# S-Taichiii/diffusion-model

Hardware: AMD Instinct MI355X
Metric: denoising steps/sec (CFG, T=1000, 32x32x4 latent, B=64) (higher is better)
Workload: dtype f32 (GEMMs: fp32 operands split fp16 hi+lo on the matrix cores, fp32 accumulate); 1 GPU; config 2: UnetCondWithGeomHead CFG=3.0 denoising step, B=64, 32x32x4, T=1000; global_batch=64, T=1000, parallelism=sample-sharded x1 (no per-step collective)

## Files before the change

diffusion-model_amd/dmx/csrc/igemm_wino.h:

```cpp
#pragma once
#include "common.h"
#include "igemm.h"
#include "igemm_x3.h"
#include "source.h"

namespace dmx {

#ifndef DMX_DIAG
#define DMX_DIAG 0
#endif
#if DMX_DIAG
constexpr int WSTAMP_SLOTS = 32, WSTAMP_BLOCKS = 2048;
__device__ unsigned long long g_wstamp[WSTAMP_SLOTS * WSTAMP_BLOCKS * 5];
DMX_DEV void wstamp(int slot, int k) {
  if (threadIdx.x == 0 && slot >= 0 && slot < WSTAMP_SLOTS) {
    const int b = (blockIdx.z * gridDim.y + blockIdx.y) * gridDim.x + blockIdx.x;
    if (b < WSTAMP_BLOCKS) {
      unsigned long long* q = g_wstamp + ((size_t)slot * WSTAMP_BLOCKS + b) * 5;
      q[k] = __builtin_amdgcn_s_memtime();
      if (k == 0) q[4] = ((unsigned long long)__builtin_amdgcn_s_getreg((20 << 0) | (0 << 6) | (3 << 11)) << 32) |
                         (unsigned)__builtin_amdgcn_s_getreg((4 << 0) | (0 << 6) | (31 << 11));
    }
  }
}
#define WSTAMP(k) wstamp(P.dslot, k)
#else
#define WSTAMP(k)
#endif

DMX_DEV double wino_u(const double (&g)[3][3], int i, int j) {
  double r[3];
#pragma unroll
  for (int b = 0; b < 3; ++b) {
    const double a0 = g[0][b], a1 = g[1][b], a2 = g[2][b];
    r[b] = i == 0 ? a0 : i == 1 ? 0.5 * (a0 + a1 + a2) : i == 2 ? 0.5 * (a0 - a1 + a2) : a2;
  }
  return j == 0 ? r[0] : j == 1 ? 0.5 * (r[0] + r[1] + r[2]) : j == 2 ? 0.5 * (r[0] - r[1] + r[2]) : r[2];
}

static __global__ void wino_pack_kernel(const float* B, int kpad, int cin, int cout, float scale, _Float16* uh,
                                        _Float16* ul) {
  const int NB = cout / 32, KK = cin / 16;
  const size_t total = (size_t)16 * NB * KK * 64;
  for (size_t q = (size_t)blockIdx.x * blockDim.x + threadIdx.x; q < total; q += (size_t)gridDim.x * blockDim.x) {
    const int lane = (int)(q & 63);
    const size_t f = q >> 6;
    const int kk = (int)(f % KK), nb = (int)((f / KK) % NB), xi = (int)(f / ((size_t)KK * NB));
    const int co = 32 * nb + (lane & 31), c0 = 16 * kk + 8 * (lane >> 5);
    half8 h, l;
#pragma unroll
    for (int e = 0; e < 8; ++e) {
      double g[3][3];
#pragma unroll
      for (int t = 0; t < 9; ++t) g[t / 3][t % 3] = (double)B[(size_t)co * kpad + (size_t)t * cin + c0 + e];
      const float u = (float)(wino_u(g, xi >> 2, xi & 3) * (double)scale);
      const _Float16 hh = (_Float16)u;
      h[e] = hh;
      l[e] = (_Float16)(u - (float)hh);
    }
    *reinterpret_cast<half8*>(uh + q * 8) = h;
    *reinterpret_cast<half8*>(ul + q * 8) = l;
  }
}

template <int W, int GNA, int EPI = EPI_STATS, int X1 = 0>
__global__ __launch_bounds__(512) void wino_kernel(const X3Params P) {
  static_assert(EPI == EPI_STATS || EPI == EPI_PARTIAL, "Winograd epilogues");
  static_assert(W == 32 || W == 16 || W == 8 || W == 4, "Winograd conv: image width 4, 8, 16 or 32");
  static_assert(W != 4 || GNA == 0, "W = 4: no GroupNorm-on-load instances");
  const IgemmParams& p = P.g;
  constexpr int TW = W / 2;
  constexpr int SPB = W == 8 ? 4 : W == 4 ? 16 : 1;
  constexpr int TPS = 64 / SPB;
  constexpr int HRS = (W == 32 ? 8 : W) + 2;
  constexpr int PS = W == 8 ? 11 : HRS;
  constexpr int HR = SPB * PS, HC = W + 2;
  constexpr int RP = W == 32 ? 88 : W == 16 ? 46 : W == 8 ? 26 : 18;
  constexpr int SQ = W == 4 ? 218 * 4 : PS * 8 * RP;
  constexpr int HBUF = SPB * SQ;
  constexpr bool RING0 = W == 4;
  constexpr int CK = 16;
  constexpr int NPC = RING0 ? SPB * W * W * (CK / 4) : HR * HC * (CK / 4);
  constexpr int NPI = (NPC + 511) / 512;
  static_assert(!RING0 || NPC % 512 == 0, "W = 4: interior pieces must fill whole thread rounds");
  constexpr int EPP = 34;
  constexpr int EPF = 16 * 32 * EPP;
  constexpr int LDSF = 2 * HBUF + 1024 > EPF ? 2 * HBUF + 1024 : EPF;
  __shared__ __attribute__((aligned(16))) float lds[LDSF];

  WSTAMP(0);
  const int tid = threadIdx.x, lane = tid & 63;
  const int wid = __builtin_amdgcn_readfirstlane(tid >> 6);
  const int wi = wid >> 1, jp = wid & 1;
  int mt, nt, bz;
  xcd_tile(mt, nt, bz);
  const int WA = p.W;
  const int BPS = W == 32 ? (p.H + 7) >> 3 : 1;
  const int HW = p.H * WA, C = p.src.C;
  const int nsmp = W == 32 ? mt / BPS : mt * SPB;
  const int band = W == 32 ? mt - nsmp * BPS : 0;
  const int y0 = 8 * band;
  const int nsamp = p.M / HW;
  const int nch_all = C / CK;
  const int cbeg = EPI == EPI_PARTIAL ? bz * p.ksplit : 0;
  const int nch = EPI == EPI_PARTIAL ? min(p.ksplit, nch_all - cbeg) : nch_all;

  int hoff[NPI], hls[NPI];
#pragma unroll
  for (int k = 0; k < NPI; ++k) {
    const int e = tid + 512 * k;
    const int h = e >> 2, q = e & 3;
    int hrow, hcol;
    if constexpr (RING0) {
      hrow = h / HC;
      hcol = h - hrow * HC;
    } else if constexpr (W == 32) {
      const int pr = (h >> 1) % 17, m = h & 1;
      hrow = (h >> 1) / 17;
      hcol = pr < 8 ? pr + 8 * m : pr < 16 ? 8 + pr + 8 * m : 32 + m;
    } else {
      const int t = (h >> 1) / HC;
      hcol = (h >> 1) - t * HC;
      hrow = 2 * t + (h & 1);
    }
    const int sh = RING0 ? h >> 4 : hrow / PS;
    const int ry = RING0 ? ((h >> 2) & 3) + 1 : hrow - sh * PS;
    const int hx = RING0 ? (h & 3) + 1 : hcol;
    const int y = y0 + ry - 1, x = hx - 1;
    const bool ok = e < NPC && ry < HRS && y >= 0 && y < p.H && x >= 0 && x < WA && nsmp + sh < nsamp;
    hoff[k] = ok ? ((((nsmp + sh) * p.H + y) * WA + x) * C + q * 4) : -1;
    hls[k] = e < NPC ? (sh * SQ + (ry * 2 + (hx & 1)) * RP * 4 + (hx >> 1) * 20 + q * 4) : 2 * HBUF + (tid & 255) * 4;
  }
  const __amdgpu_buffer_rsrc_t rA = rsrc_of(p.src.src0, P.a_bytes);
  const __amdgpu_buffer_rsrc_t rRes = rsrc_of(GNA == 2 ? (const void*)P.gn_res : (const void*)p.src.src0, P.a_bytes);

  __shared__ float2 gst_s[SPB];
  if constexpr (GNA) {
    __shared__ double gr1[4], gr2[4];
    for (int sp = 0; sp < SPB; ++sp) {
      if (tid < 256 && nsmp + sp < nsamp) {
        const float2* rp = P.gn_rowpart + (size_t)(nsmp + sp) * P.gn_cnt;
        double s1 = 0.0, s2 = 0.0;
        for (int i = tid; i < P.gn_cnt; i += 256) {
          const float2 q = rp[i];
          s1 += (double)q.x;
          s2 += (double)q.y;
        }
        s1 = wave_sum_dpp(s1);
        s2 = wave_sum_dpp(s2);
        if ((tid & 63) == 0) {
          gr1[tid >> 6] = s1;
          gr2[tid >> 6] = s2;
        }
      }
      __syncthreads();
      if (tid == 0) {
        const double cntd = (double)HW * (double)C;
        const double mean = ((gr1[0] + gr1[1]) + (gr1[2] + gr1[3])) / cntd;
        double var = ((gr2[0] + gr2[1]) + (gr2[2] + gr2[3])) / cntd - mean * mean;
        var = var < 0.0 ? 0.0 : var;
        gst_s[sp] = make_float2((float)mean, (float)(1.0 / sqrt(var + 1e-5)));
      }
      __syncthreads();
    }
  }

  floatx4 ha[NPI];
  floatx4 hr[GNA == 2 ? NPI : 1];
  auto load_halo = [&](int c) {
#pragma unroll
    for (int k = 0; k < NPI; ++k) {
      const int off = hoff[k] >= 0 ? (hoff[k] + (cbeg + c) * CK) * 4 : kOOB;
      ha[k] = bload_f4(rA, off, 0);
      if constexpr (GNA == 2) hr[k] = bload_f4(rRes, off, 0);
    }
  };
  auto store_halo = [&](int buf, int c) {
    float* hb = lds + buf * HBUF;
    floatx4 ggam = {0.f, 0.f, 0.f, 0.f}, gbet = {0.f, 0.f, 0.f, 0.f};
    if constexpr (GNA) {
      const int ch = (cbeg + c) * CK + (tid & 3) * 4;
      ggam = ld4(P.gn_gamma + ch);
      gbet = ld4(P.gn_beta + ch);
    }
#pragma unroll
    for (int k = 0; k < NPI; ++k) {
      floatx4 v = ha[k];
      if constexpr (GNA) {
        const float2 gst = gst_s[SPB == 1 ? 0 : min(hls[k] / SQ, SPB - 1)];
        v = gn_apply4v(v, gst, ggam, gbet, GNA == 1 ? 1 : 0);
        if constexpr (GNA == 2) {
#pragma unroll
          for (int j = 0; j < 4; ++j) v[j] = gelu(hr[k][j] + v[j]);
        }
        if (hoff[k] < 0) v = floatx4{0.f, 0.f, 0.f, 0.f};
      }
      *reinterpret_cast<floatx4*>(hb + hls[k]) = v;
    }
  };

  const int xi0 = 4 * wi + 2 * jp;
  const int NB = p.Cout / 32, KK = C / 16;
  const __amdgpu_buffer_rsrc_t rUh = rsrc_of(P.Uh, P.u_bytes), rUl = rsrc_of(P.Ul, P.u_bytes);
  int ub[2][2];
#pragma unroll
  for (int q = 0; q < 2; ++q)
#pragma unroll
    for (int n = 0; n < 2; ++n) ub[q][n] = (((xi0 + q) * NB + 2 * nt + n) * KK) * 1024;
  const int voff = lane * 16;
  half8 bh[2][2], bl[2][2];
  int cnext = 0;
  auto load_b = [&](int q, int n, int c) {
    const int cc = c < 0 ? cnext : c;
    bh[q][n] = bload_h8(rUh, voff, ub[q][n] + (cbeg + cc) * 1024);
    if constexpr (!X1) bl[q][n] = bload_h8(rUl, voff, ub[q][n] + (cbeg + cc) * 1024);
  };

  const int ra = wi == 0 ? 0 : wi == 2 ? 2 : 1;
  const int rb = wi == 0 ? 2 : wi == 2 ? 1 : wi == 1 ? 2 : 3;
  const float sr = wi == 1 ? 1.f : -1.f;
  const int cp = jp ? 2 : 0, cq = jp ? 1 : 2, cs = jp ? 3 : 1;
  const float sb = jp ? -1.f : 1.f;
  auto coff = [&](int col) { return (col & 1) * RP * 4 + (col >> 1) * 20; };
  const int oa = ra * 8 * RP, ob = rb * 8 * RP;
  const int op = coff(cp), oq = coff(cq), os = coff(cs);
  const int fr = lane & 31, fh = lane >> 5;
  int tb[2];
#pragma unroll
  for (int mb = 0; mb < 2; ++mb) {
    const int t = 32 * mb + fr, st = t / TPS, tt = t - st * TPS, ty = tt / TW, tx = tt - ty * TW;
    tb[mb] = st * SQ + 2 * ty * 8 * RP + tx * 20 + 8 * fh;
  }
  half8 ah[2][2], al[2][2];
  auto build = [&](int buf, int mb) {
    const float* hb = lds + buf * HBUF + tb[mb];
    unsigned vh[2][4], vl[2][4];
#pragma unroll
    for (int h = 0; h < 2; ++h) {
      floatx4 T[3];
      const int oc[3] = {op, oq, os};
#pragma unroll
      for (int k = 0; k < 3; ++k) {
        const floatx4 da = *reinterpret_cast<const floatx4*>(hb + oa + oc[k] + 4 * h);
        const floatx4 db = *reinterpret_cast<const floatx4*>(hb + ob + oc[k] + 4 * h);
#pragma unroll
        for (int e = 0; e < 4; ++e) T[k][e] = fmaf(db[e], sr, da[e]);
      }
#pragma unroll
      for (int e = 0; e < 4; e += 2) {
        const float a0 = T[0][e] - T[1][e], a1 = T[0][e + 1] - T[1][e + 1];
        const float b0 = fmaf(T[2][e], sb, T[1][e]), b1 = fmaf(T[2][e + 1], sb, T[1][e + 1]);
        if constexpr (X1) {
          vh[0][2 * h + e / 2] = __builtin_bit_cast(unsigned, __builtin_convertvector((f32x2){a0, a1}, half2v));
          vh[1][2 * h + e / 2] = __builtin_bit_cast(unsigned, __builtin_convertvector((f32x2){b0, b1}, half2v));
        } else {
          split2u(a0, a1, vh[0][2 * h + e / 2], vl[0][2 * h + e / 2]);
          split2u(b0, b1, vh[1][2 * h + e / 2], vl[1][2 * h + e / 2]);
        }
      }
    }
#pragma unroll
    for (int q = 0; q < 2; ++q) {
      ah[mb][q] = __builtin_bit_cast(half8, (u32x4){vh[q][0], vh[q][1], vh[q][2], vh[q][3]});
      if constexpr (!X1) al[mb][q] = __builtin_bit_cast(half8, (u32x4){vl[q][0], vl[q][1], vl[q][2], vl[q][3]});
    }
  };

  floatx16 acc[2][2][2];
#pragma unroll
  for (int q = 0; q < 2; ++q)
#pragma unroll
    for (int i = 0; i < 2; ++i)
#pragma unroll
      for (int j = 0; j < 2; ++j)
#pragma unroll
        for (int r = 0; r < 16; ++r) acc[q][i][j][r] = 0.f;

  if constexpr (RING0) {
    for (int i = tid; i < 2 * HBUF / 4; i += 512) *reinterpret_cast<floatx4*>(lds + 4 * i) = floatx4{0.f, 0.f, 0.f, 0.f};
  }
  load_halo(0);
  if constexpr (RING0) __syncthreads();
  store_halo(0, 0);
  load_halo(min(1, nch - 1));
  __builtin_amdgcn_sched_barrier(0);
#pragma unroll
  for (int q = 0; q < 2; ++q)
#pragma unroll
    for (int n = 0; n < 2; ++n) load_b(q, n, 0);
  __syncthreads();
  WSTAMP(1);

  auto mfmas = [&](int i, bool reload) {
#pragma unroll
    for (int q = 0; q < 2; ++q)
#pragma unroll
      for (int n = 0; n < 2; ++n) {
        if constexpr (!X1) {
          acc[q][i][n] = __builtin_amdgcn_mfma_f32_32x32x16_f16(al[i][q], bh[q][n], acc[q][i][n], 0, 0, 0);
          acc[q][i][n] = __builtin_amdgcn_mfma_f32_32x32x16_f16(ah[i][q], bl[q][n], acc[q][i][n], 0, 0, 0);
        }
        acc[q][i][n] = __builtin_amdgcn_mfma_f32_32x32x16_f16(ah[i][q], bh[q][n], acc[q][i][n], 0, 0, 0);
        if (reload) {
          load_b(q, n, -1);
          __builtin_amdgcn_sched_barrier(0x0086);
        }
      }
  };
  if constexpr (GNA == 0) {
  constexpr int NM = X1 ? 4 : 12;
  floatx4 pda[2][3], pdb[2][3], pT[3];
  u32x4 pah[2][2], pal[2][2];
  auto p_read = [&](int buf, int mb, int h) {
    const float* hb = lds + buf * HBUF + tb[mb];
    const int oc[3] = {op, oq, os};
#pragma unroll
    for (int k = 0; k < 3; ++k) {
      pda[h][k] = *reinterpret_cast<const floatx4*>(hb + oa + oc[k] + 4 * h);
      pdb[h][k] = *reinterpret_cast<const floatx4*>(hb + ob + oc[k] + 4 * h);
    }
  };
  auto p_T = [&](int h) {
#pragma unroll
    for (int k = 0; k < 3; ++k)
#pragma unroll
      for (int e = 0; e < 4; ++e) pT[k][e] = fmaf(pdb[h][k][e], sr, pda[h][k][e]);
  };
  auto p_V = [&](int mb, int h, int e) {
    const float a0 = pT[0][e] - pT[1][e], a1 = pT[0][e + 1] - pT[1][e + 1];
    const float b0 = fmaf(pT[2][e], sb, pT[1][e]), b1 = fmaf(pT[2][e + 1], sb, pT[1][e + 1]);
    const int j = 2 * h + e / 2;
    if constexpr (X1) {
      pah[mb][0][j] = __builtin_bit_cast(unsigned, __builtin_convertvector((f32x2){a0, a1}, half2v));
      pah[mb][1][j] = __builtin_bit_cast(unsigned, __builtin_convertvector((f32x2){b0, b1}, half2v));
    } else {
      unsigned h0, l0, h1, l1;
      split2u(a0, a1, h0, l0);
      split2u(b0, b1, h1, l1);
      pah[mb][0][j] = h0;
      pal[mb][0][j] = l0;
      pah[mb][1][j] = h1;
      pal[mb][1][j] = l1;
    }
  };
  auto p_piece = [&](int s, int buf, int mb) {
    if constexpr (X1) {
      if (s == 0) { p_read(buf, mb, 0); p_read(buf, mb, 1); }
      if (s == 1) { p_T(0); p_V(mb, 0, 0); p_V(mb, 0, 2); }
      if (s == 2) { p_T(1); p_V(mb, 1, 0); p_V(mb, 1, 2); }
    } else {
      if (s == 0) p_read(buf, mb, 0);
      if (s == 3) { p_T(0); p_read(buf, mb, 1); }
      if (s == 4) p_V(mb, 0, 0);
      if (s == 5) p_V(mb, 0, 2);
      if (s == 6) p_T(1);
      if (s == 7) p_V(mb, 1, 0);
      if (s == 8) p_V(mb, 1, 2);
    }
  };
  auto p_mfma = [&](int i, int s) {
    const int pr = X1 ? 2 : s % 3, qn = X1 ? s : s / 3, q = qn >> 1, n = qn & 1;
    const half8 A = __builtin_bit_cast(half8, pr == 0 ? pal[i][q] : pah[i][q]);
    const half8 Bf = pr == 1 ? bl[q][n] : bh[q][n];
    acc[q][i][n] = __builtin_amdgcn_mfma_f32_32x32x16_f16(A, Bf, acc[q][i][n], 0, 0, 0);
  };
  p_read(0, 0, 0);
  p_T(0);
  p_read(0, 0, 1);
  p_V(0, 0, 0);
  p_V(0, 0, 2);
  p_T(1);
  p_V(0, 1, 0);
  p_V(0, 1, 2);
  constexpr bool LATE = GNA == 2 || (W != 32 && GNA == 1);
  auto iter = [&](int c, auto last) {
    store_halo((c + 1) & 1, min(c + 1, nch - 1));
    if constexpr (!LATE) load_halo(min(c + 2, nch - 1));
    __builtin_amdgcn_sched_barrier(0);
#pragma unroll
    for (int sl = 0; sl < NM; ++sl) {
      p_mfma(0, sl);
      p_piece(sl, c & 1, 1);
      __builtin_amdgcn_sched_barrier(0);
    }
    __syncthreads();
    if constexpr (LATE) load_halo(min(c + 2, nch - 1));
    cnext = min(c + 1, nch - 1);
    __builtin_amdgcn_sched_barrier(0);
#pragma unroll
    for (int sl = 0; sl < NM; ++sl) {
      p_mfma(1, sl);
      if constexpr (!decltype(last)::value) p_piece(sl, (c + 1) & 1, 0);
      if (X1 || sl % 3 == 2) {
        const int qn = X1 ? sl : sl / 3;
        load_b(qn >> 1, qn & 1, -1);
      }
      __builtin_amdgcn_sched_barrier(0);
    }
  };
  for (int c = 0; c < nch - 1; ++c) iter(c, std::false_type{});
  iter(nch - 1, std::true_type{});
  } else {
  for (int c = 0; c < nch; ++c) {
    store_halo((c + 1) & 1, min(c + 1, nch - 1));
    constexpr bool LATE = GNA == 2 || (W != 32 && GNA == 1);
    if constexpr (!LATE) {
      load_halo(min(c + 2, nch - 1));
      __builtin_amdgcn_sched_barrier(0x0086);
    }
    build(c & 1, 0);
    mfmas(0, false);
    if constexpr (LATE) {
      load_halo(min(c + 2, nch - 1));
      __builtin_amdgcn_sched_barrier(0x0086);
    }
    build(c & 1, 1);
    cnext = min(c + 1, nch - 1);
    mfmas(1, true);
    __syncthreads();
  }
  }

  __syncthreads();
  WSTAMP(2);
  const int HW16 = BPS * 64 / SPB / 4, nseg = p.Cout / 32;
  const int tile0 = band * 64;
  const int cc = tid & 31, tp = tid >> 5;
#pragma unroll
  for (int mb = 0; mb < 2; ++mb)
#pragma unroll
    for (int n = 0; n < 2; ++n) {
#pragma unroll
      for (int q = 0; q < 2; ++q)
#pragma unroll
        for (int k = 0; k < 4; ++k) {
          floatx4 v;
#pragma unroll
          for (int e = 0; e < 4; ++e) v[e] = acc[q][mb][n][4 * k + e] * P.inv_scale;
          float* e = &lds[((xi0 + q) * 32 + fr) * EPP + 8 * k + 4 * fh];
          *reinterpret_cast<f32x2*>(e) = f32x2{v[0], v[1]};
          *reinterpret_cast<f32x2*>(e + 2) = f32x2{v[2], v[3]};
        }
      __syncthreads();
      float m[16][2];
#pragma unroll
      for (int xi = 0; xi < 16; ++xi) {
        const f32x2 v = *reinterpret_cast<const f32x2*>(&lds[(xi * 32 + cc) * EPP + 2 * tp]);
        m[xi][0] = v.x;
        m[xi][1] = v.y;
      }
      const int col = 64 * nt + 32 * n + cc;
      const float bias = (EPI == EPI_STATS && p.bias != nullptr) ? p.bias[col] : 0.f;
      float* dst = EPI == EPI_PARTIAL ? p.partial + (size_t)bz * p.M * p.Cout : p.out;
      float s1 = 0.f, s2 = 0.f;
#pragma unroll
      for (int e = 0; e < 2; ++e) {
        float z[4][2];
#pragma unroll
        for (int i = 0; i < 4; ++i) {
          z[i][0] = (m[4 * i][e] + m[4 * i + 1][e]) + m[4 * i + 2][e];
          z[i][1] = (m[4 * i + 1][e] - m[4 * i + 2][e]) - m[4 * i + 3][e];
        }
        const int t = 32 * mb + 2 * tp + e, st = t / TPS, tt = t - st * TPS, ty = tt / TW, tx = tt - ty * TW;
#pragma unroll
        for (int r = 0; r < 2; ++r)
#pragma unroll
          for (int s = 0; s < 2; ++s) {
            const float y = (r == 0 ? (z[0][s] + z[1][s]) + z[2][s] : (z[1][s] - z[2][s]) - z[3][s]) + bias;
            const int oy = y0 + 2 * ty + r, ox = 2 * tx + s;
            const bool in = oy < p.H && ox < WA;
            if (nsmp + st < nsamp && in)
              __builtin_nontemporal_store(y, &dst[(((size_t)(nsmp + st) * p.H + oy) * WA + ox) * p.Cout + col]);
            const float yv = in ? y : 0.f;
            s1 += yv;
            s2 += yv * yv;
          }
      }
      if constexpr (EPI == EPI_STATS) {
        s1 = wave_sum_dpp(s1);
        s2 = wave_sum_dpp(s2);
      }
      if (EPI == EPI_STATS && lane == 0) {
        const int t = 32 * mb + 4 * wid, st = t / TPS, g = (tile0 + t - st * TPS) / 4;
        if (nsmp + st < nsamp) p.rowpart[((size_t)(nsmp + st) * HW16 + g) * nseg + 2 * nt + n] = make_float2(s1, s2);
      }
      __syncthreads();
    }
  WSTAMP(3);
}

}
```

Baseline: 483.9 CFG batch-steps/s (B=64 per GPU; 2 U-Net forwards + update each).

## Extend software-pipelined Winograd main loop to GroupNorm-fused prologue variants

Enables the interleaved MFMA/transform pipeline path for GroupNorm-applied input variants (except W==8 non-X1), slicing the GN affine, GELU and LDS store of the next halo into pieces interleaved with MFMAs. GN gamma/beta loads are hoisted out of store_halo and prefetched a chunk ahead. The intent is to hide the GN apply and halo stores behind matrix-core work instead of running them serially. This adds register pressure from the extra live halo and affine state, and makes the schedule more complex, including a shifted transform start (B0) for GN variants.

```diff
diff --git a/diffusion-model_amd/dmx/csrc/igemm_wino.h b/diffusion-model_amd/dmx/csrc/igemm_wino.h
--- a/diffusion-model_amd/dmx/csrc/igemm_wino.h
+++ b/diffusion-model_amd/dmx/csrc/igemm_wino.h
@@ -165,8 +165,17 @@
     }
   }
 
+  constexpr bool PIPE = GNA == 0 || X1 || W != 8;
   floatx4 ha[NPI];
   floatx4 hr[GNA == 2 ? NPI : 1];
+  floatx4 ggam = {0.f, 0.f, 0.f, 0.f}, gbet = {0.f, 0.f, 0.f, 0.f};
+  auto load_affine = [&](int c) {
+    if constexpr (GNA) {
+      const int ch = (cbeg + c) * CK + (tid & 3) * 4;
+      ggam = ld4(P.gn_gamma + ch);
+      gbet = ld4(P.gn_beta + ch);
+    }
+  };
   auto load_halo = [&](int c) {
 #pragma unroll
     for (int k = 0; k < NPI; ++k) {
@@ -175,14 +184,8 @@
       if constexpr (GNA == 2) hr[k] = bload_f4(rRes, off, 0);
     }
   };
-  auto store_halo = [&](int buf, int c) {
+  auto store_halo = [&](int buf) {
     float* hb = lds + buf * HBUF;
-    floatx4 ggam = {0.f, 0.f, 0.f, 0.f}, gbet = {0.f, 0.f, 0.f, 0.f};
-    if constexpr (GNA) {
-      const int ch = (cbeg + c) * CK + (tid & 3) * 4;
-      ggam = ld4(P.gn_gamma + ch);
-      gbet = ld4(P.gn_beta + ch);
-    }
 #pragma unroll
     for (int k = 0; k < NPI; ++k) {
       floatx4 v = ha[k];
@@ -280,9 +283,11 @@
     for (int i = tid; i < 2 * HBUF / 4; i += 512) *reinterpret_cast<floatx4*>(lds + 4 * i) = floatx4{0.f, 0.f, 0.f, 0.f};
   }
   load_halo(0);
+  load_affine(0);
   if constexpr (RING0) __syncthreads();
-  store_halo(0, 0);
+  store_halo(0);
   load_halo(min(1, nch - 1));
+  if constexpr (PIPE) load_affine(min(1, nch - 1));
   __builtin_amdgcn_sched_barrier(0);
 #pragma unroll
   for (int q = 0; q < 2; ++q)
@@ -307,7 +312,7 @@
         }
       }
   };
-  if constexpr (GNA == 0) {
+  if constexpr (PIPE) {
   constexpr int NM = X1 ? 4 : 12;
   floatx4 pda[2][3], pdb[2][3], pT[3];
   u32x4 pah[2][2], pal[2][2];
@@ -372,15 +377,37 @@
   p_T(1);
   p_V(0, 1, 0);
   p_V(0, 1, 2);
-  constexpr bool LATE = GNA == 2 || (W != 32 && GNA == 1);
+  constexpr int NGE = NPI * 4;
+  constexpr int GS = X1 ? NM : 6;
+  constexpr int B0 = X1 || GNA == 0 ? 0 : 3;
+  constexpr int GL = X1 ? NM - 1 : 9;
+  float2 pgst;
+  constexpr bool LATE = GNA != 0 && W == 8;
+  auto g_piece = [&](int s, int buf, int cn) {
+    if (s < 0 || s >= GS) return;
+#pragma unroll
+    for (int el = s * NGE / GS; el < (s + 1) * NGE / GS; ++el) {
+      const int k = el >> 2, j = el & 3;
+      if (j == 0) pgst = gst_s[SPB == 1 ? 0 : min(hls[k] / SQ, SPB - 1)];
+      const float y = (ha[k][j] - pgst.x) * pgst.y * ggam[j] + gbet[j];
+      ha[k][j] = hoff[k] < 0 ? 0.f : gelu(GNA == 2 ? hr[k][j] + y : y);
+      if (j == 3) {
+        *reinterpret_cast<floatx4*>(lds + buf * HBUF + hls[k]) = ha[k];
+        if constexpr (!LATE) ha[k] = bload_f4(rA, hoff[k] >= 0 ? (hoff[k] + (cbeg + cn) * CK) * 4 : kOOB, 0);
+      }
+    }
+  };
   auto iter = [&](int c, auto last) {
-    store_halo((c + 1) & 1, min(c + 1, nch - 1));
-    if constexpr (!LATE) load_halo(min(c + 2, nch - 1));
+    if constexpr (GNA == 0) {
+      store_halo((c + 1) & 1);
+      load_halo(min(c + 2, nch - 1));
+    }
     __builtin_amdgcn_sched_barrier(0);
 #pragma unroll
     for (int sl = 0; sl < NM; ++sl) {
       p_mfma(0, sl);
-      p_piece(sl, c & 1, 1);
+      p_piece(sl - B0, c & 1, 1);
+      if constexpr (GNA != 0 && !decltype(last)::value) g_piece(sl, (c + 1) & 1, min(c + 2, nch - 1));
       __builtin_amdgcn_sched_barrier(0);
     }
     __syncthreads();
@@ -391,6 +418,7 @@
     for (int sl = 0; sl < NM; ++sl) {
       p_mfma(1, sl);
       if constexpr (!decltype(last)::value) p_piece(sl, (c + 1) & 1, 0);
+      if (sl == GL) load_affine(min(c + 2, nch - 1));
       if (X1 || sl % 3 == 2) {
         const int qn = X1 ? sl : sl / 3;
         load_b(qn >> 1, qn & 1, -1);
@@ -402,7 +430,8 @@
   iter(nch - 1, std::true_type{});
   } else {
   for (int c = 0; c < nch; ++c) {
-    store_halo((c + 1) & 1, min(c + 1, nch - 1));
+    load_affine(min(c + 1, nch - 1));
+    store_halo((c + 1) & 1);
     constexpr bool LATE = GNA == 2 || (W != 32 && GNA == 1);
     if constexpr (!LATE) {
       load_halo(min(c + 2, nch - 1));
```

Measured after the change: 485.6 CFG batch-steps/s (B=64 per GPU; 2 U-Net forwards + update each) (median of 6 runs). About the same (+0.4%).
